# KingOfTheAce2/video-restoration-pipeline-framewright

Measured on AMD Instinct MI355X. Metric: frames/sec Real-ESRGAN x4 1080p (RRDBNet-x4plus, 1920x1080 -> 7680x4320), higher is better.
Workload: dtype f16; 1 GPU; RealESRGAN_x4plus x4, 1920x1080 uint8 BGR frames resident in HBM -> 7680x4320 uint8 BGR in HBM, seeded synthetic weights, 43 frames per GPU

## Files before the change

video-restoration-pipeline-framewright_amd/csrc/conv3x3_mfma.hip:

```cpp
#include <mutex>
#include <cstdlib>
#include "fw_internal.h"
#include "conv_common.h"

namespace fw {

template <typename T, int CT, int EPI>
__global__ __launch_bounds__(64 * NWAVES, WAVES_PER_SIMD) void conv3x3_mfma_kernel(const ConvParams p_in) {
    ConvParams p = p_in;
    if constexpr (EPI == EPI_STORE || EPI == EPI_RESIDUAL) {
        if (p_in.n_groups > 1) {
            const int g = blockIdx.y;
            p.wpk = reinterpret_cast<const char*>(p_in.wpk) + (size_t)g * p_in.wpk_gstride;
            p.bias = p_in.bias + 32 * CT * g;
            if (p_in.chan_scale) p.chan_scale = p_in.chan_scale + 32 * CT * g;
            p.out_coff = p_in.out_coff + 32 * CT * g;
            p.f32_coff = p_in.f32_coff + 32 * CT * g;
            if (p_in.f32_native) {
                const size_t gs = (size_t)g * p_in.f32_gstride;
                if (p_in.res1) p.res1 = p_in.res1 + gs;
                if (p_in.res2) p.res2 = p_in.res2 + gs;
                if (p_in.out_f32) p.out_f32 = p_in.out_f32 + gs;
            }
        }
    }
    using SM = Smem<CT>;
    __shared__ __attribute__((aligned(16))) uint4 lds[SM::TOTAL];
    constexpr int NA = SM::NA;
    constexpr int NW = 2 * CT;

    const int tid = threadIdx.x;
    const int wave = __builtin_amdgcn_readfirstlane(tid >> 6);
    const int lane = tid & 63;
    const int q = lane & 15;
    const int sl = lane >> 4;
    constexpr bool SPLIT = EPI == EPI_RESIDUAL_SPLIT;
    FW_STAMP_INIT();

    const TileBand band;
    const int tiles_x = (p.W + TILE_W - 1) / TILE_W;
    const int tiles_y = (p.H + TILE_H - 1) / TILE_H;
    const int ntiles = tiles_x * tiles_y;
    int t_lo, t_hi;
    band.range(ntiles, &t_lo, &t_hi);
    if (t_lo >= t_hi) return;
    const int nch = p.cin_chunks;
    const int nitems = (t_hi - t_lo) * nch;

    const int ups = p.upsample2x;
    const int Ws = ups ? (p.W >> 1) : p.W;
    unsigned relb[ACT_ITERS];
    auto piece_pos = [&](int i, int* row, int* px) {
        const int idx = (ACT_ITERS * wave + i) * 64 + lane;
        const HaloPiece h = halo_piece(idx);
        *px = h.px;
        *row = (idx < ACT_PIECES) ? h.row : -1;
    };
#pragma unroll
    for (int i = 0; i < ACT_ITERS; ++i) {
        const HaloPiece h = halo_piece((ACT_ITERS * wave + i) * 64 + lane);
        const int srow = ups ? (((h.row - 1) >> 1) + 1) : h.row;
        const int spx = ups ? (((h.px - 1) >> 1) + 1) : h.px;
        relb[i] = (unsigned)(((srow * Ws + spx) * p.in_cstride + h.s * 8) * 2) + (unsigned)(4 - i % 5) * 1024u;
    }
    const unsigned lds_base = (unsigned)(size_t)(lds_ptr_t)lds;
    const char* in = reinterpret_cast<const char*>(p.in);
    const char* w_b = reinterpret_cast<const char*>(p.wpk);
    const unsigned lane16 = lane * 16;
    const long chunk_bytes = p.in_pstride * 2;

// ... 67 lines not shown
    f32x4 acc[RPW][NW][2];

    auto add_identity = [&](const uint4 (&xf)[RPW][2], float sc, int c2) {
#pragma unroll
        for (int ctl = 0; ctl < 2; ++ctl) {
            float e[8];
#pragma unroll
            for (int j = 0; j < 8; ++j) e[j] = ((id_mask >> (8 * ctl + j)) & 1u) ? sc : 0.f;
            const uint2 lo4 = Op<T>::pack4(e[0], e[1], e[2], e[3]);
            const uint2 hi4 = Op<T>::pack4(e[4], e[5], e[6], e[7]);
            const uint4 idf = make_uint4(lo4.x, lo4.y, hi4.x, hi4.y);
#pragma unroll
            for (int row = 0; row < RPW; ++row)
#pragma unroll
                for (int ph = 0; ph < 2; ++ph) {
                    if (c2)
                        acc[row][NW - 2 + ctl][ph] = Op<T>::mfma16(idf, xf[row][ph], acc[row][NW - 2 + ctl][ph]);
                    else
                        acc[row][ctl][ph] = Op<T>::mfma16(idf, xf[row][ph], acc[row][ctl][ph]);
                }
        }
    };

    issue_w(0, 0);
    issue_act();
    if (NA == 3 && nitems > 1) issue_act();

#ifndef FW_CONV_DEBUG
#define FW_CONV_DEBUG 0
#endif
    constexpr int dbg = FW_CONV_DEBUG;
    int n = 0;
    for (int t = t_lo; t < t_hi; ++t) {
        int tty, ttx;
        tile_pos(t, tiles_x, tiles_y, &tty, &ttx);
        const int y0 = tty * TILE_H;
        const int x0 = ttx * TILE_W;
#pragma unroll
        for (int w = 0; w < NW; ++w) {
            const f32x4 bv = *reinterpret_cast<const f32x4*>(p.bias + 16 * w + 4 * sl);
#pragma unroll
            for (int row = 0; row < RPW; ++row)
#pragma unroll
                for (int ph = 0; ph < 2; ++ph) acc[row][w][ph] = bv;
        }
        FW_STAMP(4);

        for (int c = 0; c < nch; ++c, ++n) {
            if (c > 0 || t == t_lo) {
                if (NA == 3 && n + 1 < nitems)
                    FW_WAIT_VMCNT(ACT_ITERS);
                else
                    FW_WAIT_VMCNT(0);
            }
            FW_STAMP(5);
            __syncthreads();
            FW_STAMP(0);
            const bool do_w = n + 1 < nitems && !(dbg & 2);
            const bool do_a = n + NA - 1 < nitems && !(dbg & 2);
            const int c1 = (c + 1 == nch) ? 0 : c + 1;
            uint4 idx[RPW][2];
            const bool has_id = SPLIT && c < p.n_id;
            auto load_residual = [&]() {
                if constexpr (SPLIT) {
                    if (has_id) {
                        const char* plane = reinterpret_cast<const char*>(p.in) + p.chunk_off[c];
#pragma unroll
                        for (int row = 0; row < RPW; ++row)
#pragma unroll
                            for (int ph = 0; ph < 2; ++ph) {
                                const int y = y0 + RPW * wave + row, x = x0 + 16 * ph + q;
                                {
                                    const char* px = (y < p.H && x < p.W) ? plane + (((size_t)y * p.W + x) * p.in_cstride + 8 * sl) * 2
                                                                          : reinterpret_cast<const char*>(p.zeros);
                                    idx[row][ph] = *reinterpret_cast<const uint4*>(px);
                                }
                            }
                    }
                }
            };
// ... 10 lines not shown
#define FW_RES_SLOT 20
#endif
            auto dma_slot = [&](int d) {
                if (d == (young ? FW_DMA_SLOT_W2 : FW_DMA_SLOT_W)) {
                    if (do_w) issue_w(c1, (n + 1) & 1);
                } else if (d == (young ? FW_DMA_SLOT_A2 : FW_DMA_SLOT_A)) {
                    if (do_a) issue_act();
                } else if (d == FW_RES_SLOT) {
                    load_residual();
                }
            };

            const uint4* a = lds + (n % NA) * ACT_REGION;
            const uint4* wl = lds + SM::W_BASE + (n & 1) * SM::W_REGION + lane;
            auto& slot_fn = dma_slot;
            conv_item<T, NW, 0>(
                acc, a, wl, rd_off, [](int tap, int w) { return tap * NW + w; }, slot_fn,
                [&](const uint4 (&xc)[RPW][2]) {
                    if constexpr (SPLIT) {
                        if (c < CT && p.in_id_scale != 0.f) add_identity(xc, p.in_id_scale, c);
                    }
                },
                [](int) {});
            FW_STAMP(1);
            if constexpr (SPLIT) {
                if (has_id) {
                    add_identity(idx, p.id_scale[c], c & 1);
                }
            }
            FW_STAMP(2);
        }

        if (NA == 3 && n + 1 < nitems)
            FW_WAIT_VMCNT(ACT_ITERS);
        else
            FW_WAIT_VMCNT(0);
        FW_STAMP(5);
        if (dbg & 4) continue;
        if constexpr (EPI == EPI_IMAGE) {
#pragma unroll
            for (int row = 0; row < RPW; ++row)
#pragma unroll
                for (int ph = 0; ph < 2; ++ph) {
                    const int y = y0 + RPW * wave + row;
                    const int x = x0 + 16 * ph + q;
                    if (sl == 0 && y < p.img_H && x < p.img_W && y < p.H && x < p.W) {
                        const size_t pix = (size_t)y * p.img_W + x;
                        const float cr = acc[row][0][ph][0], cg = acc[row][0][ph][1], cb = acc[row][0][ph][2];
                        if (p.out_rgb) {
                            float* o = p.out_rgb + pix * 3;
                            o[0] = cr;
                            o[1] = cg;
                            o[2] = cb;
                        }
                        if (p.out_u16) {
                            uint16_t* o = p.out_u16 + pix * 3;
                            o[0] = (uint16_t)rintf(fminf(fmaxf(cb, 0.f), 1.f) * 65535.f);
                            o[1] = (uint16_t)rintf(fminf(fmaxf(cg, 0.f), 1.f) * 65535.f);
                            o[2] = (uint16_t)rintf(fminf(fmaxf(cr, 0.f), 1.f) * 65535.f);
                        }
                        if (p.out_u8) {
                            uint8_t* o = p.out_u8 + pix * 3;
                            o[0] = (uint8_t)rintf(fminf(fmaxf(cb, 0.f), 1.f) * 255.f);
                            o[1] = (uint8_t)rintf(fminf(fmaxf(cg, 0.f), 1.f) * 255.f);
                            o[2] = (uint8_t)rintf(fminf(fmaxf(cr, 0.f), 1.f) * 255.f);
                        }
                    }
                }
        } else {
            constexpr int NC = 32 * CT;
            if constexpr (SPLIT) {
#pragma unroll
                for (int row = 0; row < RPW; ++row)
#pragma unroll
                    for (int w = 0; w < NW; ++w)
#pragma unroll
                        for (int ph = 0; ph < 2; ++ph) {
                            f32x4 o = acc[row][w][ph] * p.s1;
                            if (p.post_act) {
#pragma unroll
                                for (int j = 0; j < 4; ++j) o[j] = fmaxf(o[j], 0.2f * o[j]);
                            }
                            acc[row][w][ph] = o;
                        }
            } else {
#pragma unroll
                for (int row = 0; row < RPW; ++row)
#pragma unroll
                    for (int w = 0; w < NW; ++w)
#pragma unroll
                        for (int ph = 0; ph < 2; ++ph) {
// ... 9 lines not shown
                            if constexpr (EPI == EPI_RESIDUAL) {
                                if (fok) {
                                    if (p.chan_scale) o = o * *reinterpret_cast<const f32x4*>(p.chan_scale + 16 * w + 4 * sl);
                                    o = o * p.s1 + *reinterpret_cast<const f32x4*>(p.res1 + fo);
                                    if (p.res2) o = o * p.s2 + *reinterpret_cast<const f32x4*>(p.res2 + fo);
                                    if (p.post_act) {
#pragma unroll
                                        for (int j = 0; j < 4; ++j) o[j] = fmaxf(o[j], 0.2f * o[j]);
                                    }
                                }
                            } else {
                                if (p.act == 1) {
                                    o = lrelu4(o);
                                } else if (p.act == 2) {
                                    const f32x4 sl4 = *reinterpret_cast<const f32x4*>(p.chan_scale + 16 * w + 4 * sl);
#pragma unroll
                                    for (int j = 0; j < 4; ++j) o[j] = o[j] > 0.f ? o[j] : sl4[j] * o[j];
                                }
                            }
                            if (p.out_f32 && fok) *reinterpret_cast<f32x4*>(p.out_f32 + fo) = o;
                            acc[row][w][ph] = o;
                        }
            }
            FW_STAMP(3);
            if (p.out) {
                const int npass = (CT == 2 && p.out_lo) ? 2 : 1;
                const int ls = (sl & 1) ? 2 + (sl >> 1) : (sl >> 1);
                for (int pass = 0; pass < npass; ++pass) {
                    char* lane_base = reinterpret_cast<char*>(pass ? p.out_lo : p.out) +
                                      ((long)q * p.out_cstride + p.out_coff + ls * 8) * 2;
#pragma unroll
                    for (int row = 0; row < RPW; ++row) {
                        const int y = y0 + RPW * wave + row;
                        if (y >= p.H) continue;
                        const long rowoff = ((long)y * p.W + x0) * p.out_cstride * 2;
#pragma unroll
                        for (int ph = 0; ph < 2; ++ph)
#pragma unroll
                            for (int c2 = 0; c2 < CT; ++c2) {
                                f32x4 oa = acc[row][2 * c2][ph], ob = acc[row][2 * c2 + 1][ph];
                                if (pass) {
                                    oa = oa - Op<T>::unpack4(Op<T>::pack4(oa[0], oa[1], oa[2], oa[3]));
                                    ob = ob - Op<T>::unpack4(Op<T>::pack4(ob[0], ob[1], ob[2], ob[3]));
                                }
                                const uint4 v = pair16<T>(oa, ob);
                                if (x0 + 16 * ph + q < p.W)
                                    store16(lane_base + rowoff + (long)(16 * ph) * p.out_cstride * 2 + (long)c2 * p.out_pstride * 2, v);
                            }
                    }
                }
            }
            FW_STAMP(6);
        }
    }
    if constexpr (CT == 2 && (EPI == EPI_RESIDUAL || SPLIT)) FW_STAMP_FLUSH(p.stamps);
}

#undef FW_SB

#ifdef FW_PAIR_STAMP
unsigned long long* stamp_buffer(int which) {
    static unsigned long long* buf[2] = {nullptr, nullptr};
    if (!buf[which]) {
        FW_HIP_CHECK(hipMalloc((void**)&buf[which], 1024));
        FW_HIP_CHECK(hipMemset(buf[which], 0, 1024));
    }
    return buf[which];
}
extern "C" int fw_debug_stamps(int which, unsigned long long* out) {
    if (which < 0 || which > 1) return 1;
    if (hipMemcpy(out, stamp_buffer(which), 1024, hipMemcpyDeviceToHost) != hipSuccess) return 3;
    (void)hipMemset(stamp_buffer(which), 0, 1024);
    return 0;
}
#endif

static_assert(ACT_ITERS % 5 == 0, "activation pieces go out in batches of five");

static const void* zero_page() {
    static std::mutex mu;
    static void* pages[64] = {};
    int dev = 0;
    FW_HIP_CHECK(hipGetDevice(&dev));
    if (dev < 0 || dev >= 64) throw Error(1, "conv3x3: device ordinal out of range");
    std::lock_guard<std::mutex> lk(mu);
    if (!pages[dev]) {
        void* z = nullptr;
        FW_HIP_CHECK(hipMalloc(&z, 256));
        FW_HIP_CHECK(hipMemset(z, 0, 256));
        FW_HIP_CHECK(hipDeviceSynchronize());
        pages[dev] = z;
    }
    return pages[dev];
}

// ... 30 lines not shown
    if (cout_tiles == 1 && epi == EPI_STORE)
        hipLaunchKernelGGL((conv3x3_mfma_kernel<T, 1, EPI_STORE>), grid, block, 0, stream, p);
    else if (cout_tiles == 2 && epi == EPI_STORE)
        hipLaunchKernelGGL((conv3x3_mfma_kernel<T, 2, EPI_STORE>), grid, block, 0, stream, p);
    else if (cout_tiles == 2 && epi == EPI_RESIDUAL)
        hipLaunchKernelGGL((conv3x3_mfma_kernel<T, 2, EPI_RESIDUAL>), grid, block, 0, stream, p);
    else if (cout_tiles == 1 && epi == EPI_RESIDUAL)
        hipLaunchKernelGGL((conv3x3_mfma_kernel<T, 1, EPI_RESIDUAL>), grid, block, 0, stream, p);
    else if (cout_tiles == 2 && epi == EPI_RESIDUAL_SPLIT)
        hipLaunchKernelGGL((conv3x3_mfma_kernel<T, 2, EPI_RESIDUAL_SPLIT>), grid, block, 0, stream, p);
    else if (cout_tiles == 1 && epi == EPI_IMAGE)
        hipLaunchKernelGGL((conv3x3_mfma_kernel<T, 1, EPI_IMAGE>), grid, block, 0, stream, p);
    else
        throw Error(1, "conv3x3: unsupported (cout_tiles, epilogue) combination");
    FW_HIP_CHECK(hipGetLastError());
}

void launch_conv3x3(DType dt, int cout_tiles, ConvEpilogue epi, const ConvParams& p_in, hipStream_t stream) {
    ConvParams p = p_in;
    p.zeros = zero_page();
#ifdef FW_PAIR_STAMP
    p.stamps = stamp_buffer(1);
#endif


    if (p.H <= 0 || p.W <= 0 || p.cin_chunks <= 0) throw Error(1, "conv3x3: empty problem");
    if (p.upsample2x && ((p.H | p.W) & 1)) throw Error(1, "conv3x3: upsample2x needs even output size");
    if (p.in_cstride < 32 || (p.in_cstride & 7) || p.in_pstride < 32 || (p.in_pstride & 7) ||
        (p.in_pstride == 32 && p.in_cstride < 32 * p.cin_chunks &&
         (long)(p.upsample2x ? p.H / 2 : p.H) * (p.upsample2x ? p.W / 2 : p.W) > 1))
        throw Error(1, "conv3x3: bad input channel/plane stride");
    if (p.out && cout_tiles == 2 && (p.out_pstride < 32 || (p.out_pstride & 7)))
        throw Error(1, "conv3x3: bad output plane stride");
    if (p.out && ((p.out_cstride & 7) || (p.out_coff & 7))) throw Error(1, "conv3x3: output slice must be 16-byte aligned");
    if (p.act == 2 && !p.chan_scale) throw Error(1, "conv3x3: PReLU needs its slopes");
    if (p.n_groups > 1 && ((epi != EPI_STORE && epi != EPI_RESIDUAL) || p.n_groups > 64 || p.wpk_gstride <= 0 || (p.wpk_gstride & 15) || (p.f32_native && p.f32_gstride < (long)f32_native_elems(p.H, p.W, cout_tiles))))
        throw Error(1, "conv3x3: output-channel groups need EPI_STORE / EPI_RESIDUAL and a 16-byte weight stride");
    if (p.out_lo && (cout_tiles != 2 || !p.out || epi == EPI_IMAGE)) throw Error(1, "conv3x3: out_lo needs a 64-channel typed output");
    if (epi == EPI_RESIDUAL_SPLIT) {
        if (cout_tiles != 2 || p.upsample2x || !p.out || p.n_id < 0 || p.n_id > 6 || p.n_id > p.cin_chunks)
            throw Error(1, "conv3x3: bad split-trunk residual problem");
        for (int i = 0; i < p.n_id; ++i)
            if (operand_to_f32(dt, f32_to_operand(dt, p.id_scale[i])) != p.id_scale[i])
                throw Error(1, "conv3x3: identity scale not representable in the operand type");
        if (operand_to_f32(dt, f32_to_operand(dt, p.in_id_scale)) != p.in_id_scale)
            throw Error(1, "conv3x3: in_id_scale not representable in the operand type");
// ... 54 lines not shown
```

video-restoration-pipeline-framewright_amd/csrc/conv3x3_wino.hip:

```cpp
#include <cstdlib>
#include <cstring>
#include <type_traits>
#include "fw_internal.h"
#include "conv_common.h"

namespace fw {

constexpr int WN_ROWP = 2 * 17 * 4;
constexpr int WN_ACT = HALO_H * WN_ROWP;
constexpr int WN_ACT_REGION = ACT_INSTR * 64;
constexpr int WN_WFR = 3 * 4 * 4;
constexpr int WN_W_REGION = WN_WFR * 64;
constexpr int WN_TOTAL = WN_ACT_REGION + 2 * WN_W_REGION;
static_assert(NWAVES == 8 && RPW == 2 && WN_TOTAL * 16 <= 160 * 1024, "written for 8 waves of 2 rows");

typedef _Float16 wn_h2 __attribute__((ext_vector_type(2)));
__device__ __forceinline__ uint4 wn_sub(uint4 a, uint4 b) {
    uint4 r;
    r.x = __builtin_bit_cast(unsigned, __builtin_bit_cast(wn_h2, a.x) - __builtin_bit_cast(wn_h2, b.x));
    r.y = __builtin_bit_cast(unsigned, __builtin_bit_cast(wn_h2, a.y) - __builtin_bit_cast(wn_h2, b.y));
    r.z = __builtin_bit_cast(unsigned, __builtin_bit_cast(wn_h2, a.z) - __builtin_bit_cast(wn_h2, b.z));
    r.w = __builtin_bit_cast(unsigned, __builtin_bit_cast(wn_h2, a.w) - __builtin_bit_cast(wn_h2, b.w));
    return r;
}
__device__ __forceinline__ uint4 wn_add(uint4 a, uint4 b) {
    uint4 r;
    r.x = __builtin_bit_cast(unsigned, __builtin_bit_cast(wn_h2, a.x) + __builtin_bit_cast(wn_h2, b.x));
    r.y = __builtin_bit_cast(unsigned, __builtin_bit_cast(wn_h2, a.y) + __builtin_bit_cast(wn_h2, b.y));
    r.z = __builtin_bit_cast(unsigned, __builtin_bit_cast(wn_h2, a.z) + __builtin_bit_cast(wn_h2, b.z));
    r.w = __builtin_bit_cast(unsigned, __builtin_bit_cast(wn_h2, a.w) + __builtin_bit_cast(wn_h2, b.w));
    return r;
}

__device__ __forceinline__ void wn_glds_w6(const void* sbase, unsigned voff, unsigned lds_piece4) {
    const unsigned long long b = (unsigned long long)sbase;
    const unsigned long long sb = ((unsigned long long)(unsigned)__builtin_amdgcn_readfirstlane((unsigned)(b >> 32)) << 32) |
// ... 3 lines not shown
        "s_nop 4\n\t"
        "s_mov_b32 m0, %2\n\t"
        "s_nop 0\n\t"
        "global_load_lds_dwordx4 %0, %1 offset:-4096\n\t"
        "global_load_lds_dwordx4 %0, %1 offset:-3072\n\t"
        "global_load_lds_dwordx4 %0, %1 offset:-2048\n\t"
        "global_load_lds_dwordx4 %0, %1 offset:-1024\n\t"
        "global_load_lds_dwordx4 %0, %1\n\t"
        "global_load_lds_dwordx4 %0, %1 offset:1024"
        :
        : "v"(voff), "s"(sb), "s"(lds_piece4)
        : "memory");
}

template <bool PLANES, bool STORE>
__global__ __launch_bounds__(64 * NWAVES, WAVES_PER_SIMD) void conv3x3_wino_split_kernel(const ConvParams p) {
    using T = _Float16;
    __shared__ __attribute__((aligned(16))) uint4 lds[WN_TOTAL];
    const int tid = threadIdx.x;
    const int wave = __builtin_amdgcn_readfirstlane(tid >> 6);
    const int lane = tid & 63;
    const int j = lane & 15;
    const int sl = lane >> 4;

    const TileBand band;
    const int tiles_x = (p.W + TILE_W - 1) / TILE_W;
    const int tiles_y = (p.H + TILE_H - 1) / TILE_H;
    const int ntiles = tiles_x * tiles_y;
    int t_lo, t_hi;
    band.range(ntiles, &t_lo, &t_hi);
    if (t_lo >= t_hi) return;
    const int nch = p.cin_chunks;
    const int nitems = (t_hi - t_lo) * nch;

    unsigned relb[ACT_ITERS];
    auto piece_pos = [&](int i, int* row, int* px, int* s) {
        int idx = (ACT_ITERS * wave + i) * 64 + lane;
        if (idx >= WN_ACT) idx -= WN_ACT;
        const int rw = idx / WN_ROWP;
        const int rm = idx - rw * WN_ROWP;
        const int par = rm >= 68 ? 1 : 0;
        const int q = rm - 68 * par;
        const int ci = q >> 2;
        *row = rw;
        *px = 2 * ci + par;
        *s = (q & 3) ^ halo_swz(ci);
    };
#pragma unroll
    for (int i = 0; i < ACT_ITERS; ++i) {
        int row, px, s;
        piece_pos(i, &row, &px, &s);
        relb[i] = (unsigned)(((row * p.W + px) * p.in_cstride + s * 8) * 2) + (unsigned)(4 - i) * 1024u;
    }
    const unsigned lds_base = (unsigned)(size_t)(lds_ptr_t)lds;
    const char* in = reinterpret_cast<const char*>(p.in);
    const char* w_b = reinterpret_cast<const char*>(p.wpk);
// ... 76 lines not shown
                    acc[row][F][ctl] = Op<T>::mfma16(idf, xf[row], acc[row][F][ctl]);
            }
        }
    };

    auto add_identity1 = [&](int row, const uint4& xf, float sc, int c2, auto freq_tag) {
        constexpr int F = decltype(freq_tag)::value;
#pragma unroll
        for (int ctl = 0; ctl < 2; ++ctl) {
            asm volatile("" : "+v"(sc));
            float e[8];
#pragma unroll
            for (int k = 0; k < 8; ++k) e[k] = ((id_mask >> (8 * ctl + k)) & 1u) ? sc : 0.f;
            const uint2 lo4 = Op<T>::pack4(e[0], e[1], e[2], e[3]);
            const uint2 hi4 = Op<T>::pack4(e[4], e[5], e[6], e[7]);
            const uint4 idf = make_uint4(lo4.x, lo4.y, hi4.x, hi4.y);
            if (c2)
                acc[row][F][2 + ctl] = Op<T>::mfma16(idf, xf, acc[row][F][2 + ctl]);
            else
                acc[row][F][ctl] = Op<T>::mfma16(idf, xf, acc[row][F][ctl]);
        }
    };

    issue_w(0, 0);
    issue_act();

    int n = 0;
    for (int t = t_lo; t < t_hi; ++t) {
        int tty, ttx;
        tile_pos(t, tiles_x, tiles_y, &tty, &ttx);
        const int y0 = tty * TILE_H;
        const int x0 = ttx * TILE_W;
#pragma unroll
        for (int ct = 0; ct < 4; ++ct) {
            const f32x4 bv = *reinterpret_cast<const f32x4*>(p.bias + 16 * ct + 4 * sl);
#pragma unroll
            for (int row = 0; row < RPW; ++row) {
                acc[row][0][ct] = f32x4{0.f, 0.f, 0.f, 0.f};
                acc[row][1][ct] = bv;
                acc[row][2][ct] = f32x4{0.f, 0.f, 0.f, 0.f};
                acc[row][3][ct] = f32x4{0.f, 0.f, 0.f, 0.f};
            }
        }

        for (int c = 0; c < nch; ++c, ++n) {
            if (c > 0 || t == t_lo) FW_WAIT_VMCNT(0);
            __syncthreads();
            uint4 V[4][4];
            const bool own = !STORE && c < 2 && p.in_id_scale != 0.f;
#pragma unroll
            for (int r = 0; r < 4; ++r) {
                const uint4* row = lds + (RPW * wave + r) * WN_ROWP;
                const uint4 d0 = row[rd[0]], d1 = row[rd[1]], d2 = row[rd[2]], d3 = row[rd[3]];
                V[r][0] = wn_sub(d0, d2);
                V[r][1] = wn_add(d1, d2);
                V[r][2] = wn_sub(d2, d1);
                V[r][3] = wn_sub(d1, d3);
                if ((r == 1 || r == 2) && own) {
                    add_identity1(r - 1, d1, p.in_id_scale, c, std::integral_constant<int, 0>{});
                    add_identity1(r - 1, d2, -p.in_id_scale, c, std::integral_constant<int, 3>{});
                }
            }
            __syncthreads();
            const bool more = n + 1 < nitems;
            const int c1 = (c + 1 == nch) ? 0 : c + 1;
#ifndef FW_WN_DMA_K
#define FW_WN_DMA_K -1
#endif
            if (FW_WN_DMA_K < 0 && more) {
                issue_w(c1, (n + 1) & 1);
                issue_act();
            }
            uint4 ix0[RPW], ix1[RPW];
            const bool has_id = PLANES && c < p.n_id;
            const uint4* wl = lds + WN_ACT_REGION + (n & 1) * WN_W_REGION + lane;
#ifndef FW_WN_RING
#define FW_WN_RING 3
#endif
#ifndef FW_WN_RES_K
#define FW_WN_RES_K 17
#endif
            constexpr int RING = FW_WN_RING;
            uint4 wf[RING];
#pragma unroll
            for (int k = 0; k < RING - 1; ++k) wf[k] = wl[k * 64];
            FW_SB();
#pragma unroll
            for (int k = 0; k < WN_WFR; ++k) {
                const int dy = k / 16, f = (k / 4) & 3, ct = k & 3;
                if (k + RING - 1 < WN_WFR) wf[(k + RING - 1) % RING] = wl[(k + RING - 1) * 64];
                FW_SB();
                acc[0][f][ct] = Op<T>::mfma16(wf[k % RING], V[dy][f], acc[0][f][ct]);
                acc[1][f][ct] = Op<T>::mfma16(wf[k % RING], V[dy + 1][f], acc[1][f][ct]);
                FW_SB();
                if (k == FW_WN_DMA_K && more) {
                    issue_w(c1, (n + 1) & 1);
                    issue_act();
                    FW_SB();
                }
                if constexpr (PLANES) {
                    if (k == FW_WN_RES_K) {
                        const char* plane = reinterpret_cast<const char*>(p.in) + p.chunk_off[has_id ? c : 0];
#pragma unroll
                        for (int row = 0; row < RPW; ++row) {
                            const int y = y0 + RPW * wave + row, x = x0 + 2 * j;
                            const int cy = y < p.H ? y : p.H - 1, cx0 = x < p.W ? x : p.W - 1, cx1 = x + 1 < p.W ? x + 1 : p.W - 1;
                            const unsigned rowb = (unsigned)cy * (unsigned)p.W;
                            ix0[row] = *reinterpret_cast<const uint4*>(plane + ((rowb + cx0) * (unsigned)p.in_cstride + 8 * sl) * 2u);
                            ix1[row] = *reinterpret_cast<const uint4*>(plane + ((rowb + cx1) * (unsigned)p.in_cstride + 8 * sl) * 2u);
                        }
                        FW_SB();
                    }
                }
            }
            if constexpr (PLANES) {
                if (has_id) {
#pragma unroll
                    for (int row = 0; row < RPW; ++row) {
                        const int y = y0 + RPW * wave + row, x = x0 + 2 * j;
                        if (!(y < p.H && x < p.W)) ix0[row] = make_uint4(0, 0, 0, 0);
                        if (!(y < p.H && x + 1 < p.W)) ix1[row] = make_uint4(0, 0, 0, 0);
                    }
                    add_identity(ix0, p.id_scale[c], c & 1, std::integral_constant<int, 0>{});
                    add_identity(ix1, -p.id_scale[c], c & 1, std::integral_constant<int, 3>{});
                }
            }
        }

        FW_WAIT_VMCNT(0);
        const int ls = (sl & 1) ? 2 + (sl >> 1) : (sl >> 1);
        const int npass = (!STORE && p.out_lo) ? 2 : 1;
#pragma unroll
        for (int row = 0; row < RPW; ++row) {
            const int y = y0 + RPW * wave + row;
            if (y >= p.H) continue;
#pragma unroll
            for (int ct = 0; ct < 4; ++ct) {
                f32x4 ya = acc[row][0][ct] + acc[row][1][ct] + acc[row][2][ct];
                f32x4 yb = acc[row][1][ct] - acc[row][2][ct] - acc[row][3][ct];
                if constexpr (STORE) {
                    if (p.act == 1) {
                        ya = lrelu4(ya);
                        yb = lrelu4(yb);
                    }
                } else {
                    ya = ya * p.s1;
                    yb = yb * p.s1;
                }
                acc[row][0][ct] = ya;
                acc[row][3][ct] = yb;
            }
            for (int pass = 0; pass < npass; ++pass) {
                char* lane_base = reinterpret_cast<char*>(pass ? p.out_lo : p.out) + ((long)(2 * j) * p.out_cstride + p.out_coff + ls * 8) * 2;
                const long rowoff = ((long)y * p.W + x0) * p.out_cstride * 2;
#pragma unroll
                for (int e = 0; e < 2; ++e)
#pragma unroll
                    for (int c2 = 0; c2 < 2; ++c2) {
                        f32x4 oa = e ? acc[row][3][2 * c2] : acc[row][0][2 * c2], ob = e ? acc[row][3][2 * c2 + 1] : acc[row][0][2 * c2 + 1];
                        if (pass) {
                            oa = oa - Op<T>::unpack4(Op<T>::pack4(oa[0], oa[1], oa[2], oa[3]));
                            ob = ob - Op<T>::unpack4(Op<T>::pack4(ob[0], ob[1], ob[2], ob[3]));
                        }
                        const uint4 v = pair16<T>(oa, ob);
                        if (x0 + 2 * j + e < p.W) store16(lane_base + rowoff + (long)e * p.out_cstride * 2 + (long)c2 * p.out_pstride * 2, v);
                    }
            }
        }
    }
}

#undef FW_SB

size_t pack_conv3x3_wino_weights(DType dt, const float* w, int cout, int cin, int cin_chunks, uint16_t* dst) {
    const size_t n = (size_t)cin_chunks * WN_WFR * 64 * 8;
    if (!dst) return n;
    size_t o = 0;
    for (int c = 0; c < cin_chunks; ++c)
        for (int dy = 0; dy < 3; ++dy)
            for (int f = 0; f < 4; ++f)
                for (int ct = 0; ct < 4; ++ct)
                    for (int lane = 0; lane < 64; ++lane)
                        for (int e = 0; e < 8; ++e) {
                            const int co = 16 * ct + (lane & 15), ci = 32 * c + 8 * (lane >> 4) + e;
                            float u = 0.f;
                            if (co < cout && ci < cin) {
                                const float* g = w + ((size_t)co * cin + ci) * 9 + dy * 3;
                                u = f == 0 ? g[0] : f == 1 ? 0.5f * ((g[0] + g[1]) + g[2]) : f == 2 ? 0.5f * ((g[0] - g[1]) + g[2]) : g[2];
                            }
                            dst[o++] = f32_to_operand(dt, u);
                        }
    return n;
// ... 10 lines not shown
    if (p.chan_scale) throw Error(1, "conv3x3_wino: chan_scale is not implemented");
    if (p.res1 || p.res2) throw Error(1, "conv3x3_wino: fp32 residuals (res1 / res2) are not implemented");
    if (p.out_f32) throw Error(1, "conv3x3_wino: the fp32 output copy (out_f32) is not implemented");
    if (p.n_groups > 1) throw Error(1, "conv3x3_wino: output-channel groups (n_groups > 1) are not implemented");
    if (split) {
        if (p.act != 0) throw Error(1, "conv3x3_wino: no activation in the split-trunk form");
        if (p.n_id < 0 || p.n_id > 6 || p.n_id > p.cin_chunks) throw Error(1, "conv3x3_wino: bad number of residual planes (n_id)");
        if (p.n_id > 0 && (long)p.H * p.W * p.in_cstride * 2 > 0xffffffffL) throw Error(1, "conv3x3_wino: residual planes larger than 4 GiB");
        if (operand_to_f32(DT_F16, f32_to_operand(DT_F16, p.in_id_scale)) != p.in_id_scale)
            throw Error(1, "conv3x3_wino: in_id_scale not representable in f16");
        for (int i = 0; i < p.n_id; ++i)
            if (operand_to_f32(DT_F16, f32_to_operand(DT_F16, p.id_scale[i])) != p.id_scale[i])
                throw Error(1, "conv3x3_wino: identity scale not representable in f16");
    } else {
        if (p.act < 0 || p.act > 1) throw Error(1, "conv3x3_wino: act must be 0 or 1 (PReLU is not implemented)");
        if (p.n_id || p.out_lo) throw Error(1, "conv3x3_wino: residual planes / lo planes need the split-trunk form");
    }
}

void launch_conv3x3_wino_split(const ConvParams& p_in, hipStream_t stream) {
    check_conv3x3_wino(p_in, true);
    ConvParams p = p_in;
    p.zeros = conv_zero_page();
    const int tiles = ((p.W + TILE_W - 1) / TILE_W) * ((p.H + TILE_H - 1) / TILE_H);
    const int cus = conv_num_cus();
    dim3 grid(tiles < cus ? tiles : cus), block(64 * NWAVES);
    if (p.n_id > 0)
        hipLaunchKernelGGL((conv3x3_wino_split_kernel<true, false>), grid, block, 0, stream, p);
    else
        hipLaunchKernelGGL((conv3x3_wino_split_kernel<false, false>), grid, block, 0, stream, p);
    FW_HIP_CHECK(hipGetLastError());
}

void launch_conv3x3_wino_store(const ConvParams& p_in, hipStream_t stream) {
    check_conv3x3_wino(p_in, false);
    ConvParams p = p_in;
    p.zeros = conv_zero_page();
    const int tiles = ((p.W + TILE_W - 1) / TILE_W) * ((p.H + TILE_H - 1) / TILE_H);
    const int cus = conv_num_cus();
    dim3 grid(tiles < cus ? tiles : cus), block(64 * NWAVES);
    hipLaunchKernelGGL((conv3x3_wino_split_kernel<false, true>), grid, block, 0, stream, p);
    FW_HIP_CHECK(hipGetLastError());
}

}
```

video-restoration-pipeline-framewright_amd/csrc/conv_common.h:

```cpp
#pragma once
#include "fw_internal.h"

namespace fw {

typedef float f32x16 __attribute__((ext_vector_type(16)));
typedef float f32x4 __attribute__((ext_vector_type(4)));
typedef unsigned u32x2 __attribute__((ext_vector_type(2)));
typedef __bf16 bf16x8 __attribute__((ext_vector_type(8)));
typedef _Float16 f16x8 __attribute__((ext_vector_type(8)));
typedef __bf16 bf16x4 __attribute__((ext_vector_type(4)));
typedef _Float16 f16x4 __attribute__((ext_vector_type(4)));

template <typename T>
struct Op;
template <>
struct Op<__bf16> {
    static __device__ __forceinline__ f32x4 mfma16(uint4 a, uint4 b, f32x4 c) {
        return __builtin_amdgcn_mfma_f32_16x16x32_bf16(__builtin_bit_cast(bf16x8, a), __builtin_bit_cast(bf16x8, b), c, 0, 0, 0);
    }
    static __device__ __forceinline__ uint2 pack4(float a, float b, float c, float d) {
        bf16x4 v = {(__bf16)a, (__bf16)b, (__bf16)c, (__bf16)d};
        return __builtin_bit_cast(uint2, v);
    }
    static __device__ __forceinline__ f32x4 unpack4(uint2 v) {
// ... 100 lines not shown
    const int row = idx / ROWP;
    int rm = idx - row * ROWP;
    if constexpr ((ROWP & 3) != 0) rm = rm < ROWP - 1 ? rm : ROWP - 2;
    const int px = rm >> 2;
    return {row, px, (rm & 3) ^ halo_swz(px)};
}
template <int ROWP = ROW_PIECES>
__device__ __forceinline__ unsigned halo_piece_off(int idx, int W, int cstride) {
    const HaloPiece h = halo_piece<ROWP>(idx);
    return (unsigned)(((h.row * W + h.px) * cstride + h.s * 8) * 2);
}

template <int ROWP = ROW_PIECES>
__device__ __forceinline__ int halo_rd_off(int row, int px, int sl) { return row * ROWP + px * 4 + (sl ^ halo_swz(px)); }

template <int CT>
struct Smem {
    static constexpr int NA = CT == 1 ? 3 : 2;
    static constexpr int W_ITERS = (W_FRAGS * CT + NWAVES - 1) / NWAVES;
    static constexpr int W_REGION = W_FRAGS * CT * 64;
    static constexpr int W_BASE = NA * ACT_REGION;
    static constexpr int TOTAL = NA * ACT_REGION + 2 * W_REGION;
};

typedef __attribute__((address_space(3))) void* lds_ptr_t;

__device__ __forceinline__ unsigned long long uniform_base(const void* sbase) {
    const unsigned long long b = (unsigned long long)sbase;
    return ((unsigned long long)(unsigned)__builtin_amdgcn_readfirstlane((unsigned)(b >> 32)) << 32) |
           (unsigned long long)(unsigned)__builtin_amdgcn_readfirstlane((unsigned)b);
}
__device__ __forceinline__ void glds16(const void* sbase, unsigned voff, unsigned lds_dst) {
    const unsigned long long sb = uniform_base(sbase);
    lds_dst = __builtin_amdgcn_readfirstlane(lds_dst);
    asm volatile(
        "s_nop 4\n\t"
        "s_mov_b32 m0, %2\n\t"
        "s_nop 0\n\t"
        "global_load_lds_dwordx4 %0, %1"
        :
        : "v"(voff), "s"(sb), "s"(lds_dst)
        : "memory");
}

template <int N>
__device__ __forceinline__ void glds16_batch_w(const void* sbase, unsigned voff, unsigned lds_piece4) {
// ... 124 lines not shown
        const unsigned long long t_ = __builtin_amdgcn_s_memtime();      \
        __builtin_amdgcn_sched_barrier(0);                               \
        stamp_acc[slot] += t_ - stamp_last;                              \
        stamp_last = t_;                                                 \
    } while (0)
#define FW_STAMP_FLUSH(buf)                                                                       \
    do {                                                                                          \
        stamp_acc[7] = __builtin_amdgcn_s_memrealtime() - stamp_rt0;                              \
        if ((threadIdx.x & 63) == 0 && (buf)) {                                                   \
            for (int k_ = 0; k_ < 8; ++k_) atomicAdd((buf) + (threadIdx.x >> 6) * 8 + k_, stamp_acc[k_]); \
             \
                   \
            atomicMax((buf) + 64 + (threadIdx.x >> 6), stamp_acc[7]);                             \
            atomicAdd((buf) + 72 + (threadIdx.x >> 6), stamp_acc[7] * stamp_acc[7]);              \
        }                                                                                         \
    } while (0)
unsigned long long* stamp_buffer(int which);
#else
#define FW_STAMP_INIT() do { } while (0)
#define FW_STAMP(slot) do { } while (0)
#define FW_STAMP_FLUSH(buf) do { } while (0)
#endif

#define FW_WAIT_VMCNT(n)                                   \
    do {                                                   \
        __builtin_amdgcn_s_waitcnt(0x0F70 | (n));          \
        asm volatile("" ::: "memory");                     \
    } while (0)

#ifdef FW_NO_SB
#define FW_SB()
#else
#define FW_SB() __builtin_amdgcn_sched_barrier(0)
#endif

template <int ROWP, typename T, int NW, int W_LO, typename WIdx, typename Slot, typename Centre, typename Hook>
__device__ __forceinline__ void conv_item_rp(f32x4 (&acc)[RPW][NW][2], const uint4* a, const uint4* wl, const int (&rd_off)[3][2],
                                             WIdx widx, Slot dma_slot, Centre on_centre, Hook step_hook) {
    constexpr int NWU = NW - W_LO;
    constexpr int NK = 9 * NWU;
    uint4 xr[RPW + 2][2];
#ifndef FW_WRING
#define FW_WRING 3
#endif
    constexpr int RING = FW_WRING;
    uint4 wf[RING];
// ... 61 lines not shown
```

video-restoration-pipeline-framewright_amd/csrc/conv_up2x_phase.hip:

```cpp
#include <cstdlib>
#include <vector>
#include "fw_internal.h"
#include "conv_common.h"

#ifndef FW_UP_SLOT_W
#define FW_UP_SLOT_W 2
#define FW_UP_SLOT_A 6
#endif
#ifndef FW_UP_FULL_LINES
#define FW_UP_FULL_LINES 1
#endif

namespace fw {

constexpr int UP_WFRAGS = 32;
struct UpSmem {
    static constexpr int W_REGION = UP_WFRAGS * 64;
    static constexpr int W_BASE = 2 * ACT_REGION;
    static constexpr int TOTAL = 2 * ACT_REGION + 2 * W_REGION;
};
static_assert(NWAVES == 8 && RPW == 2 && ACT_ITERS == 5, "written for 8 waves of 2 rows");
static_assert(UpSmem::TOTAL * 16 <= 160 * 1024, "LDS");

__host__ __device__ constexpr int up_tx(int s) { return s < 2 ? 0 : (s < 6 ? 1 : 2); }
__host__ __device__ constexpr int up_r(int s) { return s < 2 ? s : (s < 6 ? (s - 2) >> 1 : s - 6); }
__host__ __device__ constexpr int up_b(int s) { return s < 2 ? 0 : (s < 6 ? (s - 2) & 1 : 1); }

template <typename T, typename Slot>
__device__ __forceinline__ void conv_item_up(f32x4 (&acc)[RPW][8][2], const uint4* a, const uint4* wl, const int (&rd_off)[3][2],
                                             Slot dma_slot) {
#ifndef FW_UP_WRING
#define FW_UP_WRING 3
#endif
    constexpr int RING = FW_UP_WRING;
    uint4 xr[4][2];
    uint4 wf[RING];
    auto slot_of = [](int tx, int h) { return h == 0 ? 0 : (tx == 0 ? h : (tx == 1 ? (h == 1 ? 3 : 1) : (h == 1 ? 2 : 3))); };
    auto load_w = [&](int k) { wf[k % RING] = wl[k * 64]; };
    auto load_x = [&](int tx, int h) {
#pragma unroll
        for (int ph = 0; ph < 2; ++ph) xr[slot_of(tx, h)][ph] = a[h * ROW_PIECES + rd_off[tx][ph]];
    };
// ... 29 lines not shown
        }
    }
}

template <typename T>
__global__ __launch_bounds__(64 * NWAVES, WAVES_PER_SIMD) void conv_up2x_phase_kernel(const ConvUpParams p) {
    using SM = UpSmem;
    __shared__ __attribute__((aligned(16))) uint4 lds[SM::TOTAL];

    const int tid = threadIdx.x;
    const int wave = __builtin_amdgcn_readfirstlane(tid >> 6);
    const int lane = tid & 63;
    const int q = lane & 15;
    const int sl = lane >> 4;

    const TileBand band;
    const int tiles_x = (p.W + TILE_W - 1) / TILE_W;
    const int tiles_y = (p.H + TILE_H - 1) / TILE_H;
    const int ntiles = tiles_x * tiles_y;
    int t_lo, t_hi;
    band.range(ntiles, &t_lo, &t_hi);
    if (t_lo >= t_hi) return;
    const int nitems = (t_hi - t_lo) * 4;

    unsigned relb[ACT_ITERS];
#pragma unroll
    for (int i = 0; i < ACT_ITERS; ++i)
        relb[i] = halo_piece_off((ACT_ITERS * wave + i) * 64 + lane, p.W, p.in_cstride) + (unsigned)(4 - i) * 1024u;
    const unsigned lds_base = (unsigned)(size_t)(lds_ptr_t)lds;
    const char* in = reinterpret_cast<const char*>(p.in);
    const char* w_b = reinterpret_cast<const char*>(p.wpk);
    const unsigned lane16 = lane * 16;
    const long chunk_bytes = p.in_pstride * 2;

    auto issue_act = [&](int t, int c) {
        int ty, tx;
        tile_pos(t, tiles_x, tiles_y, &ty, &tx);
        const int ty0 = ty * TILE_H, tx0 = tx * TILE_W;
        const char* src = in + (long)c * chunk_bytes + ((long)(ty0 - 1) * p.W + (tx0 - 1)) * p.in_cstride * 2;
        unsigned ok = 0;
#pragma unroll
        for (int i = 0; i < ACT_ITERS; ++i) {
            const int idx = (ACT_ITERS * wave + i) * 64 + lane;
            const HaloPiece h = halo_piece(idx);
            if (idx < ACT_PIECES && (unsigned)(ty0 - 1 + h.row) < (unsigned)p.H && (unsigned)(tx0 - 1 + h.px) < (unsigned)p.W) ok |= 1u << i;
        }
// ... 9 lines not shown
        }
    };
    auto issue_w = [&](int a, int c, int ws) {
        const int f4 = 4 * wave + 4;
        glds16_batch_w<4>(w_b + (size_t)((a * 2 + c) * UP_WFRAGS + f4) * 1024, lane16,
                          lds_base + (unsigned)(SM::W_BASE + ws * SM::W_REGION + f4 * 64) * 16u);
    };

    int rd_off[3][2];
#pragma unroll
    for (int tx = 0; tx < 3; ++tx)
#pragma unroll
        for (int ph = 0; ph < 2; ++ph) rd_off[tx][ph] = halo_rd_off(RPW * wave, 16 * ph + q + tx, sl);

    f32x4 acc[RPW][8][2];
    const int ls = (sl & 1) ? 2 + (sl >> 1) : (sl >> 1);
    const long Wout = 2L * p.W;
    char* outb = reinterpret_cast<char*>(p.out);
    [[maybe_unused]] const unsigned lane_off = (unsigned)((2 * q * p.out_cstride + ls * 8) * 2);
    const bool odd = (q & 1) != 0;
    const unsigned lane_off1 = (unsigned)(((odd ? 2 * q - 1 : 2 * q) * p.out_cstride + ls * 8) * 2);
    const unsigned lane_off2 = (unsigned)(((odd ? 2 * q + 1 : 2 * q + 2) * p.out_cstride + ls * 8) * 2);

    issue_w(0, 0, 0);
    issue_act(t_lo, 0);
    issue_act(t_lo, 1);

    int n = 0;
    for (int t = t_lo; t < t_hi; ++t) {
        const int A = (t - t_lo) & 1, B = A ^ 1;
        int tty, ttx;
        tile_pos(t, tiles_x, tiles_y, &tty, &ttx);
        const int y0 = tty * TILE_H, x0 = ttx * TILE_W;
#pragma clang loop unroll(disable)
        for (int j = 0; j < 4; ++j, ++n) {
            const int a = j >> 1;
            const int c = (j == 0 || j == 3) ? A : B;
            if ((j & 1) == 0) {
#pragma unroll
                for (int w = 0; w < 4; ++w) {
                    const f32x4 bv = *reinterpret_cast<const f32x4*>(p.bias + 16 * w + 4 * sl);
#pragma unroll
                    for (int row = 0; row < RPW; ++row)
#pragma unroll
                        for (int ph = 0; ph < 2; ++ph) {
                            acc[row][w][ph] = bv;
                            acc[row][4 + w][ph] = bv;
                        }
                }
            }
            if ((j & 1) == 1 || (j == 0 && t == t_lo)) FW_WAIT_VMCNT(0);
            __syncthreads();
            const bool more = n + 1 < nitems;
            const int na_ = j < 3 ? (j + 1) >> 1 : 0;
            const int nc_ = (j == 2) ? A : B;
            const bool act_next = j == 3 && t + 1 < t_hi;
            const bool act_this = j == 0 && t > t_lo;
            if (act_next) issue_act(t + 1, B);
            if (act_this) issue_act(t, B);
            auto dma_slot = [&](int d) {
                if (d == FW_UP_SLOT_W) {
                    if (more) issue_w(na_, nc_, (n + 1) & 1);
                }
            };
// ... 105 lines not shown
```

Baseline: 15.07 frames/s.

## Stage conv bias in LDS and pair winograd stores via DPP lane swap

Each conv kernel (mfma, winograd, up2x phase) now loads its bias vector once per block into a small LDS region before the main loop. Accumulators are then initialised from LDS instead of issuing a global load on every tile. The winograd epilogue exchanges packed outputs between adjacent lanes with a DPP swap, so each lane stores two column-adjacent 16-byte pieces in a different pattern. A compile-time-gated per-phase timing instrumentation (FW_CONV_STAMP) is also added but is off by default; the costs are an extra barrier at startup and slightly more LDS.

Result: no change. 15.18 frames/s (median of 6 runs) (+0.7%).

```diff
diff --git a/video-restoration-pipeline-framewright_amd/csrc/conv3x3_mfma.hip b/video-restoration-pipeline-framewright_amd/csrc/conv3x3_mfma.hip
--- a/video-restoration-pipeline-framewright_amd/csrc/conv3x3_mfma.hip
+++ b/video-restoration-pipeline-framewright_amd/csrc/conv3x3_mfma.hip
@@ -4,6 +4,12 @@
 #include "conv_common.h"
 
 namespace fw {
+
+#define FW_STAMP2(pair, conv) \
+    do {                      \
+        FW_STAMP(pair);       \
+        FW_CSTAMP(conv);      \
+    } while (0)
 
 template <typename T, int CT, int EPI>
 __global__ __launch_bounds__(64 * NWAVES, WAVES_PER_SIMD) void conv3x3_mfma_kernel(const ConvParams p_in) {
@@ -25,7 +31,8 @@
         }
     }
     using SM = Smem<CT>;
-    __shared__ __attribute__((aligned(16))) uint4 lds[SM::TOTAL];
+    __shared__ __attribute__((aligned(16))) uint4 lds[SM::TOTAL + BIAS_PIECES];
+    static_assert((SM::TOTAL + BIAS_PIECES) * 16 <= 160 * 1024 && 32 * CT * 4 <= BIAS_PIECES * 16, "LDS");
     constexpr int NA = SM::NA;
     constexpr int NW = 2 * CT;
 
@@ -36,6 +43,7 @@
     const int sl = lane >> 4;
     constexpr bool SPLIT = EPI == EPI_RESIDUAL_SPLIT;
     FW_STAMP_INIT();
+    FW_CSTAMP_INIT();
 
     const TileBand band;
     const int tiles_x = (p.W + TILE_W - 1) / TILE_W;
@@ -46,6 +54,7 @@
     if (t_lo >= t_hi) return;
     const int nch = p.cin_chunks;
     const int nitems = (t_hi - t_lo) * nch;
+    const float bias_g = bias_prefetch(p.bias, 32 * CT, tid);
 
     const int ups = p.upsample2x;
     const int Ws = ups ? (p.W >> 1) : p.W;
@@ -159,9 +168,11 @@
         }
     };
 
+    const float* bias_l = bias_stage(lds + SM::TOTAL, bias_g, 32 * CT, tid);
     issue_w(0, 0);
     issue_act();
     if (NA == 3 && nitems > 1) issue_act();
+    __syncthreads();
 
 #ifndef FW_CONV_DEBUG
 #define FW_CONV_DEBUG 0
@@ -175,13 +186,13 @@
         const int x0 = ttx * TILE_W;
 #pragma unroll
         for (int w = 0; w < NW; ++w) {
-            const f32x4 bv = *reinterpret_cast<const f32x4*>(p.bias + 16 * w + 4 * sl);
+            const f32x4 bv = *reinterpret_cast<const f32x4*>(bias_l + 16 * w + 4 * sl);
 #pragma unroll
             for (int row = 0; row < RPW; ++row)
 #pragma unroll
                 for (int ph = 0; ph < 2; ++ph) acc[row][w][ph] = bv;
         }
-        FW_STAMP(4);
+        FW_STAMP2(4, CS_SETUP);
 
         for (int c = 0; c < nch; ++c, ++n) {
             if (c > 0 || t == t_lo) {
@@ -190,9 +201,9 @@
                 else
                     FW_WAIT_VMCNT(0);
             }
-            FW_STAMP(5);
+            FW_STAMP2(5, CS_WAIT);
             __syncthreads();
-            FW_STAMP(0);
+            FW_STAMP2(0, CS_BARRIER);
             const bool do_w = n + 1 < nitems && !(dbg & 2);
             const bool do_a = n + NA - 1 < nitems && !(dbg & 2);
             const int c1 = (c + 1 == nch) ? 0 : c + 1;
@@ -249,20 +260,20 @@
                     }
                 },
                 [](int) {});
-            FW_STAMP(1);
+            FW_STAMP2(1, CS_KLOOP);
             if constexpr (SPLIT) {
                 if (has_id) {
                     add_identity(idx, p.id_scale[c], c & 1);
                 }
             }
-            FW_STAMP(2);
+            FW_STAMP2(2, CS_RESID);
         }
 
         if (NA == 3 && n + 1 < nitems)
             FW_WAIT_VMCNT(ACT_ITERS);
         else
             FW_WAIT_VMCNT(0);
-        FW_STAMP(5);
+        FW_STAMP2(5, CS_EPI_WAIT);
         if (dbg & 4) continue;
         if constexpr (EPI == EPI_IMAGE) {
 #pragma unroll
@@ -294,6 +305,7 @@
                         }
                     }
                 }
+            FW_CSTAMP(CS_STORE);
         } else {
             constexpr int NC = 32 * CT;
             if constexpr (SPLIT) {
@@ -349,7 +361,7 @@
                             acc[row][w][ph] = o;
                         }
             }
-            FW_STAMP(3);
+            FW_STAMP2(3, CS_CONVERT);
             if (p.out) {
                 const int npass = (CT == 2 && p.out_lo) ? 2 : 1;
                 const int ls = (sl & 1) ? 2 + (sl >> 1) : (sl >> 1);
@@ -375,15 +387,21 @@
                                     store16(lane_base + rowoff + (long)(16 * ph) * p.out_cstride * 2 + (long)c2 * p.out_pstride * 2, v);
                             }
                     }
+                    if (pass)
+                        FW_CSTAMP(CS_STORE_LO);
+                    else
+                        FW_CSTAMP(CS_STORE);
                 }
             }
             FW_STAMP(6);
         }
     }
     if constexpr (CT == 2 && (EPI == EPI_RESIDUAL || SPLIT)) FW_STAMP_FLUSH(p.stamps);
+    FW_CSTAMP_FLUSH(p.stamps);
 }
 
 #undef FW_SB
+#undef FW_STAMP2
 
 #ifdef FW_PAIR_STAMP
 unsigned long long* stamp_buffer(int which) {
@@ -398,6 +416,23 @@
     if (which < 0 || which > 1) return 1;
     if (hipMemcpy(out, stamp_buffer(which), 1024, hipMemcpyDeviceToHost) != hipSuccess) return 3;
     (void)hipMemset(stamp_buffer(which), 0, 1024);
+    return 0;
+}
+#endif
+
+#ifdef FW_CONV_STAMP
+unsigned long long* conv_stamp_buffer(int which) {
+    static unsigned long long* buf[2] = {nullptr, nullptr};
+    if (!buf[which]) {
+        FW_HIP_CHECK(hipMalloc((void**)&buf[which], 1024));
+        FW_HIP_CHECK(hipMemset(buf[which], 0, 1024));
+    }
+    return buf[which];
+}
+extern "C" int fw_debug_conv_stamps(int which, unsigned long long* out) {
+    if (which < 0 || which > 1) return 1;
+    if (hipMemcpy(out, conv_stamp_buffer(which), 1024, hipMemcpyDeviceToHost) != hipSuccess) return 3;
+    (void)hipMemset(conv_stamp_buffer(which), 0, 1024);
     return 0;
 }
 #endif
@@ -474,6 +509,9 @@
 #ifdef FW_PAIR_STAMP
     p.stamps = stamp_buffer(1);
 #endif
+#ifdef FW_CONV_STAMP
+    p.stamps = conv_stamp_buffer(1);
+#endif
 
 
     if (p.H <= 0 || p.W <= 0 || p.cin_chunks <= 0) throw Error(1, "conv3x3: empty problem");
diff --git a/video-restoration-pipeline-framewright_amd/csrc/conv3x3_wino.hip b/video-restoration-pipeline-framewright_amd/csrc/conv3x3_wino.hip
--- a/video-restoration-pipeline-framewright_amd/csrc/conv3x3_wino.hip
+++ b/video-restoration-pipeline-framewright_amd/csrc/conv3x3_wino.hip
@@ -11,7 +11,8 @@
 constexpr int WN_ACT_REGION = ACT_INSTR * 64;
 constexpr int WN_WFR = 3 * 4 * 4;
 constexpr int WN_W_REGION = WN_WFR * 64;
-constexpr int WN_TOTAL = WN_ACT_REGION + 2 * WN_W_REGION;
+constexpr int WN_BIAS = WN_ACT_REGION + 2 * WN_W_REGION;
+constexpr int WN_TOTAL = WN_BIAS + BIAS_PIECES;
 static_assert(NWAVES == 8 && RPW == 2 && WN_TOTAL * 16 <= 160 * 1024, "written for 8 waves of 2 rows");
 
 typedef _Float16 wn_h2 __attribute__((ext_vector_type(2)));
@@ -61,6 +62,7 @@
     const int lane = tid & 63;
     const int j = lane & 15;
     const int sl = lane >> 4;
+    FW_CSTAMP_INIT();
 
     const TileBand band;
     const int tiles_x = (p.W + TILE_W - 1) / TILE_W;
@@ -71,6 +73,7 @@
     if (t_lo >= t_hi) return;
     const int nch = p.cin_chunks;
     const int nitems = (t_hi - t_lo) * nch;
+    const float bias_g = bias_prefetch(p.bias, 64, tid);
 
     unsigned relb[ACT_ITERS];
     auto piece_pos = [&](int i, int* row, int* px, int* s) {
@@ -193,8 +196,10 @@
         }
     };
 
+    const float* bias_l = bias_stage(lds + WN_BIAS, bias_g, 64, tid);
     issue_w(0, 0);
     issue_act();
+    __syncthreads();
 
     int n = 0;
     for (int t = t_lo; t < t_hi; ++t) {
@@ -204,7 +209,7 @@
         const int x0 = ttx * TILE_W;
 #pragma unroll
         for (int ct = 0; ct < 4; ++ct) {
-            const f32x4 bv = *reinterpret_cast<const f32x4*>(p.bias + 16 * ct + 4 * sl);
+            const f32x4 bv = *reinterpret_cast<const f32x4*>(bias_l + 16 * ct + 4 * sl);
 #pragma unroll
             for (int row = 0; row < RPW; ++row) {
                 acc[row][0][ct] = f32x4{0.f, 0.f, 0.f, 0.f};
@@ -213,10 +218,13 @@
                 acc[row][3][ct] = f32x4{0.f, 0.f, 0.f, 0.f};
             }
         }
+        FW_CSTAMP(CS_SETUP);
 
         for (int c = 0; c < nch; ++c, ++n) {
             if (c > 0 || t == t_lo) FW_WAIT_VMCNT(0);
+            FW_CSTAMP(CS_WAIT);
             __syncthreads();
+            FW_CSTAMP(CS_BARRIER);
             uint4 V[4][4];
             const bool own = !STORE && c < 2 && p.in_id_scale != 0.f;
 #pragma unroll
@@ -232,6 +240,7 @@
                     add_identity1(r - 1, d2, -p.in_id_scale, c, std::integral_constant<int, 3>{});
                 }
             }
+            FW_CSTAMP(CS_READ);
             __syncthreads();
             const bool more = n + 1 < nitems;
             const int c1 = (c + 1 == nch) ? 0 : c + 1;
@@ -242,6 +251,7 @@
                 issue_w(c1, (n + 1) & 1);
                 issue_act();
             }
+            FW_CSTAMP(CS_BAR2);
             uint4 ix0[RPW], ix1[RPW];
             const bool has_id = PLANES && c < p.n_id;
             const uint4* wl = lds + WN_ACT_REGION + (n & 1) * WN_W_REGION + lane;
@@ -284,6 +294,7 @@
                     }
                 }
             }
+            FW_CSTAMP(CS_KLOOP);
             if constexpr (PLANES) {
                 if (has_id) {
 #pragma unroll
@@ -295,10 +306,12 @@
                     add_identity(ix0, p.id_scale[c], c & 1, std::integral_constant<int, 0>{});
                     add_identity(ix1, -p.id_scale[c], c & 1, std::integral_constant<int, 3>{});
                 }
+                FW_CSTAMP(CS_RESID);
             }
         }
 
         FW_WAIT_VMCNT(0);
+        FW_CSTAMP(CS_EPI_WAIT);
         const int ls = (sl & 1) ? 2 + (sl >> 1) : (sl >> 1);
         const int npass = (!STORE && p.out_lo) ? 2 : 1;
 #pragma unroll
@@ -321,24 +334,42 @@
                 acc[row][0][ct] = ya;
                 acc[row][3][ct] = yb;
             }
+            FW_CSTAMP(CS_CONVERT);
+            const bool odd = (j & 1) != 0;
+            const int col1 = odd ? 2 * j - 1 : 2 * j, col2 = col1 + 2;
             for (int pass = 0; pass < npass; ++pass) {
-                char* lane_base = reinterpret_cast<char*>(pass ? p.out_lo : p.out) + ((long)(2 * j) * p.out_cstride + p.out_coff + ls * 8) * 2;
+                char* lane_base = reinterpret_cast<char*>(pass ? p.out_lo : p.out) + ((long)col1 * p.out_cstride + p.out_coff + ls * 8) * 2;
                 const long rowoff = ((long)y * p.W + x0) * p.out_cstride * 2;
 #pragma unroll
-                for (int e = 0; e < 2; ++e)
-#pragma unroll
-                    for (int c2 = 0; c2 < 2; ++c2) {
+                for (int c2 = 0; c2 < 2; ++c2) {
+                    uint4 v[2];
+#pragma unroll
+                    for (int e = 0; e < 2; ++e) {
                         f32x4 oa = e ? acc[row][3][2 * c2] : acc[row][0][2 * c2], ob = e ? acc[row][3][2 * c2 + 1] : acc[row][0][2 * c2 + 1];
                         if (pass) {
                             oa = oa - Op<T>::unpack4(Op<T>::pack4(oa[0], oa[1], oa[2], oa[3]));
                             ob = ob - Op<T>::unpack4(Op<T>::pack4(ob[0], ob[1], ob[2], ob[3]));
                         }
-                        const uint4 v = pair16<T>(oa, ob);
-                        if (x0 + 2 * j + e < p.W) store16(lane_base + rowoff + (long)e * p.out_cstride * 2 + (long)c2 * p.out_pstride * 2, v);
+                        v[e] = pair16<T>(oa, ob);
                     }
+                    const uint4 snd = odd ? v[0] : v[1];
+                    uint4 rcv;
+                    rcv.x = (unsigned)__builtin_amdgcn_mov_dpp((int)snd.x, 0xB1, 0xF, 0xF, true);
+                    rcv.y = (unsigned)__builtin_amdgcn_mov_dpp((int)snd.y, 0xB1, 0xF, 0xF, true);
+                    rcv.z = (unsigned)__builtin_amdgcn_mov_dpp((int)snd.z, 0xB1, 0xF, 0xF, true);
+                    rcv.w = (unsigned)__builtin_amdgcn_mov_dpp((int)snd.w, 0xB1, 0xF, 0xF, true);
+                    char* dst = lane_base + rowoff + (long)c2 * p.out_pstride * 2;
+                    if (x0 + col1 < p.W) store16(dst, odd ? rcv : v[0]);
+                    if (x0 + col2 < p.W) store16(dst + (long)2 * p.out_cstride * 2, odd ? v[1] : rcv);
+                }
+                if (pass)
+                    FW_CSTAMP(CS_STORE_LO);
+                else
+                    FW_CSTAMP(CS_STORE);
             }
         }
     }
+    FW_CSTAMP_FLUSH(p.stamps);
 }
 
 #undef FW_SB
@@ -395,6 +426,9 @@
     check_conv3x3_wino(p_in, true);
     ConvParams p = p_in;
     p.zeros = conv_zero_page();
+#ifdef FW_CONV_STAMP
+    p.stamps = conv_stamp_buffer(0);
+#endif
     const int tiles = ((p.W + TILE_W - 1) / TILE_W) * ((p.H + TILE_H - 1) / TILE_H);
     const int cus = conv_num_cus();
     dim3 grid(tiles < cus ? tiles : cus), block(64 * NWAVES);
@@ -409,6 +443,9 @@
     check_conv3x3_wino(p_in, false);
     ConvParams p = p_in;
     p.zeros = conv_zero_page();
+#ifdef FW_CONV_STAMP
+    p.stamps = conv_stamp_buffer(0);
+#endif
     const int tiles = ((p.W + TILE_W - 1) / TILE_W) * ((p.H + TILE_H - 1) / TILE_H);
     const int cus = conv_num_cus();
     dim3 grid(tiles < cus ? tiles : cus), block(64 * NWAVES);
diff --git a/video-restoration-pipeline-framewright_amd/csrc/conv_common.h b/video-restoration-pipeline-framewright_amd/csrc/conv_common.h
--- a/video-restoration-pipeline-framewright_amd/csrc/conv_common.h
+++ b/video-restoration-pipeline-framewright_amd/csrc/conv_common.h
@@ -146,6 +146,14 @@
     static constexpr int W_BASE = NA * ACT_REGION;
     static constexpr int TOTAL = NA * ACT_REGION + 2 * W_REGION;
 };
+
+constexpr int BIAS_PIECES = 16;
+__device__ __forceinline__ float bias_prefetch(const float* bias, int n, int tid) { return tid < n ? bias[tid] : 0.f; }
+__device__ __forceinline__ const float* bias_stage(uint4* lds_bias, float v, int n, int tid) {
+    float* b = reinterpret_cast<float*>(lds_bias);
+    if (tid < n) b[tid] = v;
+    return b;
+}
 
 typedef __attribute__((address_space(3))) void* lds_ptr_t;
 
@@ -316,6 +324,50 @@
 #define FW_STAMP_FLUSH(buf) do { } while (0)
 #endif
 
+#ifdef FW_CONV_STAMP
+#ifdef FW_PAIR_STAMP
+#error "FW_CONV_STAMP and FW_PAIR_STAMP are two diagnostic builds"
+#endif
+enum ConvStampSlot {
+    CS_SETUP = 0,
+    CS_WAIT = 1,
+    CS_BARRIER = 2,
+    CS_READ = 3,
+    CS_BAR2 = 4,
+    CS_KLOOP = 5,
+    CS_RESID = 6,
+    CS_EPI_WAIT = 7,
+    CS_CONVERT = 8,
+    CS_STORE = 9,
+    CS_STORE_LO = 10,
+    CS_LIFE = 15
+};
+#define FW_CSTAMP_INIT()                                                                 \
+    unsigned stamp_acc[16] = {0, 0, 0, 0, 0, 0, 0, 0, 0, 0, 0, 0, 0, 0, 0, 0};           \
+    unsigned stamp_last = (unsigned)__builtin_amdgcn_s_memtime();                       \
+    const unsigned stamp_rt0 = (unsigned)__builtin_amdgcn_s_memrealtime()
+#define FW_CSTAMP(slot)                                                  \
+    do {                                                                 \
+        __builtin_amdgcn_sched_barrier(0);                               \
+        const unsigned t_ = (unsigned)__builtin_amdgcn_s_memtime();      \
+        __builtin_amdgcn_sched_barrier(0);                               \
+        stamp_acc[slot] += t_ - stamp_last;                              \
+        stamp_last = t_;                                                 \
+    } while (0)
+#define FW_CSTAMP_FLUSH(buf)                                                                                   \
+    do {                                                                                                      \
+        stamp_acc[CS_LIFE] = (unsigned)__builtin_amdgcn_s_memrealtime() - stamp_rt0;                          \
+        if ((threadIdx.x & 63) == 0 && (buf))                                                                 \
+            for (int k_ = 0; k_ < 16; ++k_)                                                                   \
+                atomicAdd((buf) + (threadIdx.x >> 6) * 16 + k_, (unsigned long long)stamp_acc[k_]);           \
+    } while (0)
+unsigned long long* conv_stamp_buffer(int which);
+#else
+#define FW_CSTAMP_INIT() do { } while (0)
+#define FW_CSTAMP(slot) do { } while (0)
+#define FW_CSTAMP_FLUSH(buf) do { } while (0)
+#endif
+
 #define FW_WAIT_VMCNT(n)                                   \
     do {                                                   \
         __builtin_amdgcn_s_waitcnt(0x0F70 | (n));          \
diff --git a/video-restoration-pipeline-framewright_amd/csrc/conv_up2x_phase.hip b/video-restoration-pipeline-framewright_amd/csrc/conv_up2x_phase.hip
--- a/video-restoration-pipeline-framewright_amd/csrc/conv_up2x_phase.hip
+++ b/video-restoration-pipeline-framewright_amd/csrc/conv_up2x_phase.hip
@@ -17,7 +17,8 @@
 struct UpSmem {
     static constexpr int W_REGION = UP_WFRAGS * 64;
     static constexpr int W_BASE = 2 * ACT_REGION;
-    static constexpr int TOTAL = 2 * ACT_REGION + 2 * W_REGION;
+    static constexpr int BIAS = 2 * ACT_REGION + 2 * W_REGION;
+    static constexpr int TOTAL = BIAS + BIAS_PIECES;
 };
 static_assert(NWAVES == 8 && RPW == 2 && ACT_ITERS == 5, "written for 8 waves of 2 rows");
 static_assert(UpSmem::TOTAL * 16 <= 160 * 1024, "LDS");
@@ -93,6 +94,7 @@
     band.range(ntiles, &t_lo, &t_hi);
     if (t_lo >= t_hi) return;
     const int nitems = (t_hi - t_lo) * 4;
+    const float bias_g = bias_prefetch(p.bias, 64, tid);
 
     unsigned relb[ACT_ITERS];
 #pragma unroll
@@ -148,9 +150,11 @@
     const unsigned lane_off1 = (unsigned)(((odd ? 2 * q - 1 : 2 * q) * p.out_cstride + ls * 8) * 2);
     const unsigned lane_off2 = (unsigned)(((odd ? 2 * q + 1 : 2 * q + 2) * p.out_cstride + ls * 8) * 2);
 
+    const float* bias_l = bias_stage(lds + SM::BIAS, bias_g, 64, tid);
     issue_w(0, 0, 0);
     issue_act(t_lo, 0);
     issue_act(t_lo, 1);
+    __syncthreads();
 
     int n = 0;
     for (int t = t_lo; t < t_hi; ++t) {
@@ -165,7 +169,7 @@
             if ((j & 1) == 0) {
 #pragma unroll
                 for (int w = 0; w < 4; ++w) {
-                    const f32x4 bv = *reinterpret_cast<const f32x4*>(p.bias + 16 * w + 4 * sl);
+                    const f32x4 bv = *reinterpret_cast<const f32x4*>(bias_l + 16 * w + 4 * sl);
 #pragma unroll
                     for (int row = 0; row < RPW; ++row)
 #pragma unroll
```
